# symek/facedeform

Hardware: AMD Instinct MI355X
Metric: deformed Mverts/sec at 256 ctrl pts, 1/2/4/8 MI355X vs host-CPU ref (higher is better)
Workload: dtype f32

## Files before the change

### facedeform_amd/csrc/fd_eval_shared.hip

```cpp
#include <cstdio>
#include <cstdlib>

#include <type_traits>

#include "fd_eval_common.h"
#include "fd_shared_common.h"

namespace fd {

namespace {


constexpr int kSharedThreads = 512;
constexpr int kWideWaves = 8;

constexpr bool shared_dense(int nF) { return nF > 12; }
constexpr int shared_tiles(int nF) { return shared_dense(nF) ? 3 * ((nF + 15) / 16) : (nF + 3) / 4; }
constexpr int shared_slots(int nT, bool dense) { return dense ? nT / 3 * 16 : nT * 4; }


struct SharedOut {
    float *P_out[kMaxBatch];
    float *falloff_out[kMaxBatch];
};

struct SharedParams {
    int64_t N;
    const float *P_in;
    const float *dist2;
    const float *tu, *tv, *nrm;
    float radius2, falloffrate;
    int ntiles;
    int nkb;
    int nF, nT;
    int kchunk;
    const MfmaTileH *ctiles;
    const float *norm;
    const uint4 *wtiles;
    const SharedFrame *frames;
    int fast;
    int delta;
    unsigned long long *stamps;
};

struct SharedSlots {
    const Rec32 *rec32[kMaxBatch];
    const DevModel *model[kMaxBatch];
    const double *centres[kMaxBatch];
    int M;
    int nreal;
    int *mismatch;
};

__device__ __forceinline__ bool rig_matches(const SharedSlots &slots, int f, int nF, int l, int per)
{
    bool same = true;
    if (f > 0 && f < nF && slots.centres[f] != slots.centres[0]) {
        const double *a = slots.centres[f], *b0 = slots.centres[0];
        const int n = 3 * slots.M;
        bool diff = false;
        int e = l;
        for (; e + 7 * per < n; e += 8 * per) {
            double va[8], vb[8];
#pragma unroll
            for (int u = 0; u < 8; ++u) { va[u] = a[e + u * per]; vb[u] = b0[e + u * per]; }
#pragma unroll
            for (int u = 0; u < 8; ++u) diff |= !(va[u] == vb[u]);
        }
        for (; e < n; e += per) diff |= !(a[e] == b0[e]);
        same = !diff;
    }
    for (int off = per / 2; off >= 1; off >>= 1) same = (__shfl_xor((int)same, off) != 0) && same;
    if (!same && l == 0 && slots.mismatch) *slots.mismatch = (f < slots.nreal ? f : slots.nreal - 1) + 1;
    return same;
}

__global__ __launch_bounds__(256) void k_pack_shared(const SharedSlots slots, const SharedOut out, int nF, int Mpad, int dense,
                                                      uint4 *wtiles, SharedFrame *frames, const MfmaTileH *ctiles, int gauss)
{
    const int kb = blockIdx.x, T = blockIdx.y, nT = gridDim.y, nkb = gridDim.x;
    if (T == 0 && gauss) {
        constexpr int per = (int)(sizeof(MfmaTileH) / 16);
        uint4 *dst = wtiles + (size_t)nkb * nT * 128 + (size_t)nT * 64;
        if (threadIdx.x < 32) {
            const int centre = 32 * kb + (int)threadIdx.x;
            dst[(size_t)2 * kb * per + threadIdx.x] =
                centre < Mpad ? *reinterpret_cast<const uint4 *>(&slots.rec32[0][centre]) : make_uint4(0u, 0u, 0u, 0u);
        }
        if (kb == 0 && threadIdx.x == 255) {
            const float *nn = slots.model[0]->norm32;
            dst[(size_t)2 * nkb * per] = make_uint4(__float_as_uint(nn[0]), __float_as_uint(nn[1]), __float_as_uint(nn[2]), __float_as_uint(nn[3]));
        }
    } else if (T == 0) {
        constexpr int per = (int)(sizeof(MfmaTileH) / 16);
        uint4 *dst = wtiles + (size_t)nkb * nT * 128 + (size_t)nT * 64;
        const int ntiles = Mpad / 16;
        if ((int)threadIdx.x < 2 * per) {
            const int tile = 2 * kb + (int)threadIdx.x / per;
            dst[(size_t)2 * kb * per + threadIdx.x] =
                tile < ntiles ? reinterpret_cast<const uint4 *>(ctiles + tile)[threadIdx.x % per] : make_uint4(0u, 0u, 0u, 0u);
        }
        if (kb == 0 && threadIdx.x == 255) {
            const float *nn = slots.model[0]->norm32;
            dst[(size_t)2 * nkb * per] = make_uint4(__float_as_uint(nn[0]), __float_as_uint(nn[1]), __float_as_uint(nn[2]), __float_as_uint(nn[3]));
        }
    }
    const int lane = threadIdx.x & 63, g = lane >> 4, rho = lane & 15;
    const int nfr = dense ? 16 : 4, f0 = dense ? 16 * (T / 3) : 4 * T;
    const int fi = dense ? rho : rho >> 2, c = dense ? T % 3 : rho & 3;
    __shared__ float s_scale[16];
    {
        const int per = 256 / nfr, q = threadIdx.x / per, l = threadIdx.x % per;
        const int f = f0 + q;
        float m = 0.f;
        if (f < nF) {
            m = slots.model[f]->wmax32;
        }
        for (int off = per / 2; off >= 1; off >>= 1) m = fmaxf(m, __shfl_xor(m, off));
        const bool same_rig = (kb == 0 && (!dense || T % 3 == 0)) ? rig_matches(slots, f, nF, l, per) : true;
        if (l == 0) {
            int k = 0;
            if (m > 0.f && m < INFINITY) k = 13 - (__builtin_amdgcn_frexp_expf(m) - 1);
            k = k < -100 ? -100 : (k > 100 ? 100 : k);
            s_scale[q] = ldexpf(1.f, k);
            if (kb == 0 && (!dense || T % 3 == 0)) {
                SharedFrame fr;
                fr.inv_scale = ldexpf(1.f, -k - (gauss ? kGaussShift : 0));
                fr.built = (f < nF && same_rig && slots.model[f]->terminationtype == 1) ? 1 : 0;
                fr.pad[0] = fr.pad[1] = 0;
                fr.P_out = f < nF ? out.P_out[f] : nullptr;
                fr.falloff_out = f < nF ? out.falloff_out[f] : nullptr;
                frames[f] = fr;
            }
        }
    }
    __syncthreads();
    if (threadIdx.x >= 64) return;
    const int f = f0 + fi;
    const float sc = s_scale[fi];
    f16x8 hi, lo;
#pragma unroll
    for (int sidx = 0; sidx < 8; ++sidx) {
        const int centre = 32 * kb + 16 * (sidx >> 2) + 4 * g + (sidx & 3);
        float w = 0.f;
        if (f < nF && c < 3 && centre < Mpad) {
            const Rec32 r = slots.rec32[f][centre];
            w = (c == 0 ? r.wx : (c == 1 ? r.wy : r.wz)) * sc;
        }
        const _Float16 h = (_Float16)w;
        hi[sidx] = h;
        lo[sidx] = (_Float16)(w - (float)h);
    }
    uint4 *dst = wtiles + ((size_t)kb * nT + T) * 128;
    dst[lane] = __builtin_bit_cast(uint4, hi);
    dst[64 + lane] = __builtin_bit_cast(uint4, lo);
// ... 764 lines not shown
                }
            }
            phi_half(nk - 1, 1, b1h, b1l);
            contract_half(nk - 1, 0, b0h, b0l);
            contract_half(nk - 1, 1, b1h, b1l);
        }

        FD_SSTAMP(1)
#pragma unroll
        for (int c = 0; c < NT; ++c) {
#pragma unroll
            for (int r = 0; r < 16; ++r) {
                const u32x2 sw = __builtin_amdgcn_permlane32_swap(__float_as_uint(acc[c][0][r]), __float_as_uint(acc[c][1][r]), false, false);
                acc[c][0][r] = __uint_as_float(sw[0]); acc[c][1][r] = __uint_as_float(sw[1]);
            }
        }
        const int64_t i = vbase + lane;
        const bool inb = i < p.N;
        const int64_t ic = inb ? i : p.N - 1;
        const bool gated = own_d2 > p.radius2;
        const unsigned off12 = 12u * (unsigned)lane, off4 = 4u * (unsigned)lane;
        if constexpr (!FAST) {
            nxt = load_raw(gu_next, fastTag);
        }
        auto row_of = [&](int fs, int c) -> float {
            const int row = 3 * fs + c, T = row / 32, rho = row % 32;
            return acc[T][(rho % 8) / 4][4 * (rho / 8) + rho % 4];
        };
        FD_SSTAMP(2)
        if constexpr (FAST) {
            const f32x4 ones = {1.f, 1.f, 1.f, 1.f};
            const unsigned voff = 12u * (unsigned)vbase + off12;
            const uint64_t fbase = 4ull * (uint64_t)vbase;
#pragma unroll
            for (int fs = 0; fs < NSLOT; ++fs) {
                const float inv = __uint_as_float((unsigned)__builtin_amdgcn_readlane((int)tab[(8 * fs) / 64], (8 * fs) % 64));
                const uint64_t pout = ((uint64_t)(unsigned)__builtin_amdgcn_readlane((int)tab[(8 * fs + 5) / 64], (8 * fs + 5) % 64) << 32) |
                                      (unsigned)__builtin_amdgcn_readlane((int)tab[(8 * fs + 4) / 64], (8 * fs + 4) % 64);
                const float d0 = row_of(fs, 0), d1 = row_of(fs, 1), d2c = row_of(fs, 2);
                if (fs % 4 == 0) __builtin_nontemporal_store(ones, (f32x4_a16 FD_GLOBAL *)(s_ftab[(fs / 4) * 64 + lane] + fbase));
                store_pos3_nt((Pos3 FD_GLOBAL *)((char FD_GLOBAL *)pout + voff), __builtin_fmaf(d0, inv, pos[0]), __builtin_fmaf(d1, inv, pos[1]),
                              __builtin_fmaf(d2c, inv, pos[2]));
            }
            settle(nxt);
            FD_SSTAMP(3)
            return;
        }
        if (inb && gated) {
            for (int f = 0; f < p.nF; ++f) {
                float *dstp = s_frames[f].P_out;
                if (p.delta) store_pos3((Pos3 FD_GLOBAL *)as_global(dstp) + i, 0.f, 0.f, 0.f);
                else if (dstp != p.P_in) store_pos3((Pos3 FD_GLOBAL *)as_global(dstp) + i, pos[0], pos[1], pos[2]);
            }
        }
        float fall = 1.f;
        float a1[3] = {0.f, 0.f, 0.f}, a2[3] = {0.f, 0.f, 0.f};
        const bool doit = inb && !gated;
        const float base[3] = {p.delta ? 0.f : pos[0], p.delta ? 0.f : pos[1], p.delta ? 0.f : pos[2]};
        if (doit) {
            if (p.dist2 != nullptr || !(p.radius2 != 0.f)) {
                const float q = fminf(own_d2 / p.radius2, 1.f);
                fall = powf(1.f - q, p.falloffrate);
            }
            if (p.tu) {
                float u[3] = {p.tu[3 * ic], p.tu[3 * ic + 1], p.tu[3 * ic + 2]};
                float v[3] = {p.tv[3 * ic], p.tv[3 * ic + 1], p.tv[3 * ic + 2]};
                float n[3] = {p.nrm[3 * ic], p.nrm[3 * ic + 1], p.nrm[3 * ic + 2]};
                normalize3(u[0], u[1], u[2]);
                normalize3(v[0], v[1], v[2]);
                normalize3(n[0], n[1], n[2]);
                float gm[3][3];
#pragma unroll
                for (int r = 0; r < 3; ++r)
#pragma unroll
                    for (int c = 0; c < 3; ++c) gm[r][c] = u[r] * u[c] + v[r] * v[c] + n[r] * n[c];
#pragma unroll
                for (int c = 0; c < 3; ++c) {
                    a1[c] = u[0] * gm[0][c] + u[1] * gm[1][c] + u[2] * gm[2][c];
                    a2[c] = v[0] * gm[0][c] + v[1] * gm[1][c] + v[2] * gm[2][c];
                }
                normalize3(a1[0], a1[1], a1[2]);
                normalize3(a2[0], a2[1], a2[2]);
            }
        }
#pragma unroll
        for (int fs = 0; fs < NSLOT; ++fs) {
            const int f = fs;
            if (f >= p.nF) continue;
            const float inv = __uint_as_float((unsigned)__builtin_amdgcn_readlane((int)tab[(8 * f) / 64], (8 * f) % 64));
            const bool built = __builtin_amdgcn_readlane((int)tab[(8 * f + 1) / 64], (8 * f + 1) % 64) != 0;
            const uint64_t pout = ((uint64_t)(unsigned)__builtin_amdgcn_readlane((int)tab[(8 * f + 5) / 64], (8 * f + 5) % 64) << 32) |
                                  (unsigned)__builtin_amdgcn_readlane((int)tab[(8 * f + 4) / 64], (8 * f + 4) % 64);
            const uint64_t fout = ((uint64_t)(unsigned)__builtin_amdgcn_readlane((int)tab[(8 * f + 7) / 64], (8 * f + 7) % 64) << 32) |
                                  (unsigned)__builtin_amdgcn_readlane((int)tab[(8 * f + 6) / 64], (8 * f + 6) % 64);
            if (!doit) continue;
            Pos3 FD_GLOBAL *dstP = (Pos3 FD_GLOBAL *)((char FD_GLOBAL *)(pout + 12ull * (uint64_t)vbase) + off12);
            if (!built) {
                if (p.delta) store_pos3(dstP, 0.f, 0.f, 0.f);
                else if (pout != (uint64_t)p.P_in) store_pos3(dstP, pos[0], pos[1], pos[2]);
                continue;
            }
            float disp[3] = {row_of(fs, 0) * inv, row_of(fs, 1) * inv, row_of(fs, 2) * inv};
            if (p.tu) {
                const float da1 = disp[0] * a1[0] + disp[1] * a1[1] + disp[2] * a1[2];
                const float da2 = disp[0] * a2[0] + disp[1] * a2[1] + disp[2] * a2[2];
#pragma unroll
                for (int c = 0; c < 3; ++c) disp[c] = a1[c] * da1 + a2[c] * da2;
            }
            if (fout) __builtin_nontemporal_store(fall, (float FD_GLOBAL *)((char FD_GLOBAL *)(fout + 4ull * (uint64_t)vbase) + off4));
            store_pos3_nt(dstP, base[0] + disp[0] * fall, base[1] + disp[1] * fall, base[2] + disp[2] * fall);
        }
        FD_SSTAMP(3)
    };
    bool built_here = true;
#pragma unroll
    for (int q = 0; q < kTabRegs; ++q) {
        const int idx = 64 * q + lane;
        if (idx < NSLOT * 8 && (idx & 7) == 1) built_here = built_here && tab[q] != 0u;
    }
    const bool fast_ok = p.fast && __all(built_here);
    const int nfull = (int)(p.N / THREADS);
    int u = dynamic ? next_unit(0) : wave;
    int ru = dynamic ? round_taken : 0;
    nxt = load_raw(unit_group(u) < ngroups ? unit_global(u) : 0, std::false_type{});
    settle(nxt);
    if (fast_ok) {
        while (unit_group(u) < nfull) {
            const int un = next_unit(u);
            const int run = dynamic ? round_taken : ru + 1;
            do_group(u, un, ru, std::true_type{});
            u = un; ru = run;
        }
    }
    while (unit_group(u) < ngroups) {
        const int un = next_unit(u);
        const int run = dynamic ? round_taken : ru + 1;
        do_group(u, un, ru, std::false_type{});
        u = un; ru = run;
    }
    if (stamp && lane == 0 && wave < 8) {
        for (int q = 0; q < 4; ++q) p.stamps[wave * 8 + q] = st_acc[q];
        p.stamps[wave * 8 + 4] = __builtin_amdgcn_s_memtime() - st_t0;
        p.stamps[wave * 8 + 5] = __builtin_amdgcn_s_memrealtime() - st_r0;
    }
    if (p.stamps != nullptr && lane == 0 && wave < 8 && blockIdx.x < kMaxCUs) {
        p.stamps[64 + ((size_t)blockIdx.x * 8 + wave) * 2] = st_r0;
        p.stamps[64 + ((size_t)blockIdx.x * 8 + wave) * 2 + 1] = __builtin_amdgcn_s_memrealtime();
    }
#undef FD_SSTAMP
}

constexpr int kW1Waves = 12;
constexpr int kW1Unit = 32;
constexpr size_t w1_fixed_lds(int nt) { return sizeof(SharedFrame) * (size_t)kWideSlots + 32 * 16 + (size_t)nt * 64 * 16 + 256 * sizeof(uint64_t) + 16; }

template <bool GAUSS, int NT, int NSLOT>
__global__ __launch_bounds__(64 * kW1Waves) __attribute__((amdgpu_waves_per_eu(kW1Waves / 4, kW1Waves / 4)))
void k_deform32_shared_w1(const SharedParams p, int ngroups)
{
    constexpr int WAVES = kW1Waves, THREADS = 64 * WAVES;
    constexpr int NLF = NSLOT / 2;
    constexpr int NFQ = (NSLOT + 7) / 8;
    static_assert(NSLOT % 4 == 0 && NSLOT <= kWideSlots && 3 * NLF <= 16 * NT, "frame slots in fours, three rows each, half of them per lane half");
    constexpr int kW16 = wide_w16(NT);
    extern __shared__ __attribute__((aligned(16))) char smem[];
    SharedFrame *s_frames = reinterpret_cast<SharedFrame *>(smem);
    uint4 *s_ptab = reinterpret_cast<uint4 *>(smem + sizeof(SharedFrame) * (size_t)kWideSlots);
    uint4 *s_poly = s_ptab + 32;
    uint64_t *s_ftab = reinterpret_cast<uint64_t *>(s_poly + NT * 64);
    unsigned *s_ticket = reinterpret_cast<unsigned *>(s_ftab + 256);
    uint4 *s_ct = reinterpret_cast<uint4 *>(s_ticket + 4);
    uint4 *s_w = s_ct + (size_t)64 * p.kchunk;
    const int tid = threadIdx.x;
    const int lane = tid & 63;
    const int wave = __builtin_amdgcn_readfirstlane(tid >> 6);
    const int h = lane >> 5, j = lane & 31;
    const float n0 = p.norm[0], n1 = p.norm[1], n2 = p.norm[2];
    const float inv_s = p.norm[3];
    f32x16 zero16;
#pragma unroll
    for (int r = 0; r < 16; ++r) zero16[r] = 0.f;

    auto stage_model = [&]() {
        const int nk = p.nkb;
        for (int q = tid; q < nk * 64; q += THREADS) s_ct[q] = reinterpret_cast<const uint4 *>(p.ctiles)[q];
        const u32x4 *src = reinterpret_cast<const u32x4 *>(p.wtiles);
        u32x4 *dst = reinterpret_cast<u32x4 *>(s_w);
        const int n16 = nk * kW16;
        int q = tid;
        for (; q + 7 * THREADS < n16; q += 8 * THREADS) {
            const u32x4 v0 = src[q], v1 = src[q + THREADS], v2 = src[q + 2 * THREADS], v3 = src[q + 3 * THREADS];
            const u32x4 v4 = src[q + 4 * THREADS], v5 = src[q + 5 * THREADS], v6 = src[q + 6 * THREADS], v7 = src[q + 7 * THREADS];
            dst[q] = v0; dst[q + THREADS] = v1; dst[q + 2 * THREADS] = v2; dst[q + 3 * THREADS] = v3;
            dst[q + 4 * THREADS] = v4; dst[q + 5 * THREADS] = v5; dst[q + 6 * THREADS] = v6; dst[q + 7 * THREADS] = v7;
        }
        for (; q < n16; q += THREADS) dst[q] = src[q];
        __syncthreads();
    };

    {
        const uint4 *src = reinterpret_cast<const uint4 *>(p.frames);
        uint4 *dst = reinterpret_cast<uint4 *>(s_frames);
        for (int q = tid; q < kWideSlots * (int)(sizeof(SharedFrame) / 16); q += THREADS) dst[q] = src[q];
        const uint4 *psrc = p.wtiles + (size_t)p.nkb * kW16;
        for (int q = tid; q < NT * 64; q += THREADS) s_poly[q] = psrc[q];
        if (tid == 0) *s_ticket = 0u;
        if (tid < 32) {
            const SharedFrame fr = p.frames[tid < NSLOT ? tid : NSLOT - 1];
            const uint64_t po = (uint64_t)fr.P_out;
            s_ptab[tid] = make_uint4((unsigned)po, (unsigned)(po >> 32), __float_as_uint(fr.inv_scale), (unsigned)fr.built);
        }
        if (p.fast && tid < NFQ * 64) {
            const int f = 8 * (tid >> 6) + ((tid & 63) >> 3);
            s_ftab[tid] = (uint64_t)p.frames[f < NSLOT ? f : NSLOT - 1].falloff_out + 16u * (unsigned)(tid & 7);
        }
    }
    stage_model();

    struct UnitRaw { float p[3]; float d2; };
    const int whole_rounds = ngroups / (int)gridDim.x;
    const int pool0 = whole_rounds * (int)gridDim.x * WAVES, total_units = ngroups * WAVES;
    auto unit_global = [&](int u) -> int {
        if (u < WAVES * whole_rounds) return ((int)blockIdx.x + (u / WAVES) * (int)gridDim.x) * WAVES + (u % WAVES);
        const int q = u - WAVES * whole_rounds;
        return q < 2 * WAVES ? pool0 + (int)blockIdx.x + q * (int)gridDim.x : total_units;
    };
    auto unit_group = [&](int u) -> int { const int g = unit_global(u); return g < total_units ? (g / WAVES) : ngroups; };
    auto next_unit = [&](int u) {
        (void)u;
        unsigned v = 0;
        if (lane == 0) v = __hip_atomic_fetch_add(s_ticket, 1u, __ATOMIC_RELAXED, __HIP_MEMORY_SCOPE_WORKGROUP);
        return (int)__builtin_amdgcn_readfirstlane(v);
    };
    auto load_raw = [&](int gu, auto fastTag) {
        constexpr bool FAST = decltype(fastTag)::value;
        UnitRaw r;
        const int64_t vi = (int64_t)gu * kW1Unit + j;
        const int64_t vc = vi < p.N ? vi : p.N - 1;
        if constexpr (FAST) {
            const char *pb = reinterpret_cast<const char *>(p.P_in) + (size_t)(12u * (unsigned)vc);
            r.p[0] = __builtin_nontemporal_load(reinterpret_cast<const float *>(pb)); r.p[1] = __builtin_nontemporal_load(reinterpret_cast<const float *>(pb + 4));
            r.p[2] = __builtin_nontemporal_load(reinterpret_cast<const float *>(pb + 8));
            r.d2 = 0.f;
        } else {
            r.p[0] = __builtin_nontemporal_load(&p.P_in[3 * vc]); r.p[1] = __builtin_nontemporal_load(&p.P_in[3 * vc + 1]);
            r.p[2] = __builtin_nontemporal_load(&p.P_in[3 * vc + 2]);
            r.d2 = p.dist2 ? p.dist2[vc] : 0.f;
        }
        return r;
    };
    auto settle = [&](const UnitRaw &r) { asm volatile("" :: "v"(r.p[0]), "v"(r.p[1]), "v"(r.p[2])); };
    UnitRaw nxt;
    int uc = 0;
#ifdef FD_TUNING
    const bool stamp = p.stamps != nullptr && blockIdx.x == 0;
    const unsigned long long st_t0 = p.stamps ? __builtin_amdgcn_s_memtime() : 0, st_r0 = p.stamps ? __builtin_amdgcn_s_memrealtime() : 0;
    unsigned long long st_prev = st_t0, st_acc[4] = {0, 0, 0, 0};
#define FD_W1STAMP(K) if (stamp) { __builtin_amdgcn_sched_barrier(0); const unsigned long long t_ = __builtin_amdgcn_s_memtime(); st_acc[K] += t_ - st_prev; st_prev = t_; __builtin_amdgcn_sched_barrier(0); }
#else
#define FD_W1STAMP(K)
#endif
    auto do_unit = [&](int u, int un, auto fastTag) {
        constexpr bool FAST = decltype(fastTag)::value;
        const int64_t vbase = (int64_t)unit_global(u) * kW1Unit;
        const int gu_next = unit_group(un) < ngroups ? unit_global(un) : unit_global(u);
        const UnitRaw cur = nxt;
        const float pos[3] = {cur.p[0], cur.p[1], cur.p[2]};
        const float own_d2 = cur.d2;
        f32x16 acc[NT];
        const float x = (cur.p[0] - n0) * inv_s, y = (cur.p[1] - n1) * inv_s, z = (cur.p[2] - n2) * inv_s;
        const bool lane_live = FAST ? true : ((vbase + j < p.N) && !(own_d2 > p.radius2));
        const float xx = __builtin_fmaf(z, z, __builtin_fmaf(y, y, x * x));
        f16x8 bop;
        {
            const float va = h == 0 ? -2.f * x : -2.f * z, vb2 = h == 0 ? -2.f * y : xx;
            const _Float16 ha = (_Float16)va, la = (_Float16)(va - (float)ha);
            const _Float16 hb = (_Float16)vb2, lb = (_Float16)(vb2 - (float)hb);
            const _Float16 one = (_Float16)1.0f;
            bop = h == 0 ? (f16x8){ha, la, ha, la, hb, lb, hb, lb} : (f16x8){ha, la, ha, la, one, one, hb, lb};
        }
        {
            constexpr float ps = GAUSS ? (float)(1 << kGaussShift) : 1.f;
            constexpr unsigned one16 = GAUSS ? 0x6400u : 0x3c00u;
            unsigned xyh, xyl, zxh, zxl;
            split_pair_f16(x * ps, y * ps, xyh, xyl);
            split_pair_f16(z * ps, xx * ps, zxh, zxl);
            u32x4 pb;
            if (h == 0) pb = (u32x4){one16 | (xyh << 16), (xyh >> 16) | (zxh << 16), (zxh >> 16) | (xyl << 16), (xyl >> 16) | (zxl << 16)};
            else pb = (u32x4){(zxl >> 16) | (one16 << 16), xyh, zxh, 0u};
            const f16x8 pbv = __builtin_bit_cast(f16x8, pb);
#pragma unroll
            for (int c = 0; c < NT; ++c)
                acc[c] = __builtin_amdgcn_mfma_f32_32x32x16_f16(__builtin_bit_cast(f16x8, s_poly[c * 64 + lane]), pbv, zero16, 0, 0, 0);
        }
        const bool wave_work = FAST ? true : __any(lane_live);
        if constexpr (FAST) nxt = load_raw(gu_next, fastTag);
        FD_W1STAMP(0)

        f32x16 dd;
        f16x8 w0h, w0l;
        auto d2_block = [&](int kb) {
            if constexpr (!GAUSS) dd = __builtin_amdgcn_mfma_f32_32x32x16_f16(__builtin_bit_cast(f16x8, s_ct[(size_t)kb * 64 + lane]), bop, zero16, 0, 0, 0);
        };
        auto phi_from = [&](int kb, u32x8 &xh, u32x8 &xl) {
            if constexpr (GAUSS) {
                const float4 *cr = reinterpret_cast<const float4 *>(s_ct + (size_t)kb * 64) + 4 * h;
#pragma unroll
                for (int q = 0; q < 8; ++q) {
                    float ph[2];
#pragma unroll
                    for (int e = 0; e < 2; ++e) {
                        const float4 c = cr[8 * (q >> 1) + 2 * (q & 1) + e];
                        const float dx = x - c.x, dy = y - c.y, dz = z - c.z;
                        float d2 = dx * dx;
                        d2 = __builtin_fmaf(dy, dy, d2);
                        d2 = __builtin_fmaf(dz, dz, d2);
                        ph[e] = __builtin_amdgcn_exp2f(__builtin_fmaf(d2, c.w, (float)kGaussShift));
                    }
                    unsigned hh, ll;
                    split_pair_f16<true>(ph[0], ph[1], hh, ll);
                    xh[q] = hh; xl[q] = ll;
                }
            } else {
#pragma unroll
                for (int q = 0; q < 8; ++q) {
                    unsigned hh, ll;
                    split_pair_f16<false, false>(d2_log_d2(dd[2 * q]), d2_log_d2(dd[2 * q + 1]), hh, ll);
                    xh[q] = hh; xl[q] = ll;
                }
                asm volatile("s_nop 1" : "+v"(xl[0]), "+v"(xl[1]), "+v"(xl[2]), "+v"(xl[3]), "+v"(xl[4]), "+v"(xl[5]), "+v"(xl[6]), "+v"(xl[7]));
            }
        };
        auto step = [&](int kb, int nk, const u32x8 &ch, const u32x8 &cl, u32x8 &nh, u32x8 &nl, auto lastTag) {
            constexpr bool LAST = decltype(lastTag)::value;
            constexpr int NP = 2 * NT;
            const uint4 *wk = s_w + (size_t)kb * kW16 + lane;
            const int kbn = kb + 1 < nk ? kb + 1 : kb, kbd = kb + 2 < nk ? kb + 2 : nk - 1;
            const uint4 *wkn = s_w + (size_t)kbn * kW16 + lane;
            if constexpr (!LAST) phi_from(kb + 1, nh, nl);
            f16x8 ph_ = w0h, pl_ = w0l;
#pragma unroll
            for (int pr = 0; pr < NP; ++pr) {
                const int s_ = pr / NT, c = pr % NT;
                f16x8 qh, ql;
                if (pr + 1 < NP) {
                    const int s2 = (pr + 1) / NT, c2 = (pr + 1) % NT;
                    qh = __builtin_bit_cast(f16x8, wk[((c2 * 2 + s2) * 2) * 64]); ql = __builtin_bit_cast(f16x8, wk[((c2 * 2 + s2) * 2 + 1) * 64]);
                } else {
                    qh = __builtin_bit_cast(f16x8, wkn[0]); ql = __builtin_bit_cast(f16x8, wkn[64]);
                }
                const f16x8 vh = __builtin_bit_cast(f16x8, (u32x4){ch[4 * s_], ch[4 * s_ + 1], ch[4 * s_ + 2], ch[4 * s_ + 3]});
                const f16x8 vl = __builtin_bit_cast(f16x8, (u32x4){cl[4 * s_], cl[4 * s_ + 1], cl[4 * s_ + 2], cl[4 * s_ + 3]});
                acc[c] = __builtin_amdgcn_mfma_f32_32x32x16_f16(ph_, vh, acc[c], 0, 0, 0);
                if constexpr (!LAST) if (pr == NP - 1) d2_block(kbd);
                acc[c] = __builtin_amdgcn_mfma_f32_32x32x16_f16(pl_, vh, acc[c], 0, 0, 0);
                acc[c] = __builtin_amdgcn_mfma_f32_32x32x16_f16(ph_, vl, acc[c], 0, 0, 0);
                ph_ = qh; pl_ = ql;
            }
            w0h = ph_; w0l = pl_;
            if constexpr (GAUSS || LAST) return;
            constexpr int NM = 6 * NT, TR2 = NT == 3 ? 0 : 8;
            constexpr int QD = 3 * (NP - 1);
#pragma unroll
            for (int q = 0; q < NM; ++q) {
                if (q < TR2) __builtin_amdgcn_sched_group_barrier(0x400, 2, 0);
                else if (q < TR2 + (16 - 2 * TR2)) __builtin_amdgcn_sched_group_barrier(0x400, 1, 0);
                __builtin_amdgcn_sched_group_barrier(0x008, 1, 0);
                if (q % 3 == 0) __builtin_amdgcn_sched_group_barrier(0x100, 2, 0);
                if (q == 1) __builtin_amdgcn_sched_group_barrier(0x100, 1, 0);
                if (q == QD) __builtin_amdgcn_sched_group_barrier(0x008, 1, 0);
                __builtin_amdgcn_sched_group_barrier(0x002, NT == 3 ? kW1Vpm : kW1Vpm + 1, 0);
            }
        };
        const bool k_loop = FAST || wave_work;
        if (k_loop) {
            const int nk = p.nkb;
            u32x8 ah_, al_, bh_, bl_;
            d2_block(0);
            phi_from(0, ah_, al_);
            d2_block(nk > 1 ? 1 : 0);
            w0h = __builtin_bit_cast(f16x8, s_w[lane]); w0l = __builtin_bit_cast(f16x8, s_w[64 + lane]);
            int kb = 0;
            while (kb + 2 < nk) {
                step(kb, nk, ah_, al_, bh_, bl_, std::false_type{});
                step(kb + 1, nk, bh_, bl_, ah_, al_, std::false_type{});
                kb += 2;
            }
            if (kb + 2 == nk) {
                step(kb, nk, ah_, al_, bh_, bl_, std::false_type{});
                step(kb + 1, nk, bh_, bl_, ah_, al_, std::true_type{});
            } else {
                step(kb, nk, ah_, al_, bh_, bl_, std::true_type{});
            }
        }

        auto accf = [&](int k) -> float { return acc[k / 16][k % 16]; };
        const int64_t i = vbase + j;
        FD_W1STAMP(1)
        if constexpr (!FAST) nxt = load_raw(gu_next, fastTag);
        if constexpr (FAST) {
            const f32x4 ones = {1.f, 1.f, 1.f, 1.f};
            uint64_t voff = 12ull * (uint64_t)i, fbase = 4ull * (uint64_t)vbase;
            asm volatile("" : "+v"(voff));
            uint4 ent[NLF];
            uint64_t fptr[NFQ];
#pragma unroll
            for (int lf = 0; lf < NLF; ++lf) ent[lf] = s_ptab[2 * lf + h];
#pragma unroll
            for (int q = 0; q < NFQ; ++q) fptr[q] = s_ftab[q * 64 + lane];
            __builtin_amdgcn_sched_group_barrier(0x100, NLF + NFQ, 0);
#pragma unroll
            for (int lf = 0; lf < NLF; ++lf) {
                const uint4 e = ent[lf];
                const uint64_t dst = (((uint64_t)e.y << 32) | (uint64_t)e.x) + voff;
                const float inv = __uint_as_float(e.z);
                if (lf % 4 == 0) __builtin_nontemporal_store(ones, (f32x4_a16 FD_GLOBAL *)(fptr[lf / 4] + fbase));
                store_pos3_nt((Pos3 FD_GLOBAL *)dst, __builtin_fmaf(accf(3 * lf), inv, pos[0]), __builtin_fmaf(accf(3 * lf + 1), inv, pos[1]),
                              __builtin_fmaf(accf(3 * lf + 2), inv, pos[2]));
            }
            settle(nxt);
            ++uc;
            FD_W1STAMP(2)
            return;
        }
        const bool inb = i < p.N;
        const int64_t ic = inb ? i : p.N - 1;
        const bool gated = own_d2 > p.radius2;
        if (inb && gated) {
            for (int f = h; f < p.nF; f += 2) {
                float *dstp = s_frames[f].P_out;
                if (p.delta) store_pos3((Pos3 FD_GLOBAL *)as_global(dstp) + i, 0.f, 0.f, 0.f);
                else if (dstp != p.P_in) store_pos3((Pos3 FD_GLOBAL *)as_global(dstp) + i, pos[0], pos[1], pos[2]);
            }
        }
        float fall = 1.f;
        float a1[3] = {0.f, 0.f, 0.f}, a2[3] = {0.f, 0.f, 0.f};
        const bool doit = inb && !gated;
        const float base[3] = {p.delta ? 0.f : pos[0], p.delta ? 0.f : pos[1], p.delta ? 0.f : pos[2]};
        if (doit) {
            if (p.dist2 != nullptr || !(p.radius2 != 0.f)) {
                const float q = fminf(own_d2 / p.radius2, 1.f);
                fall = powf(1.f - q, p.falloffrate);
            }
            if (p.tu) {
                float u3[3] = {p.tu[3 * ic], p.tu[3 * ic + 1], p.tu[3 * ic + 2]};
                float v3[3] = {p.tv[3 * ic], p.tv[3 * ic + 1], p.tv[3 * ic + 2]};
                float n3[3] = {p.nrm[3 * ic], p.nrm[3 * ic + 1], p.nrm[3 * ic + 2]};
                normalize3(u3[0], u3[1], u3[2]);
                normalize3(v3[0], v3[1], v3[2]);
                normalize3(n3[0], n3[1], n3[2]);
                float gm[3][3];
#pragma unroll
                for (int r = 0; r < 3; ++r)
#pragma unroll
                    for (int c = 0; c < 3; ++c) gm[r][c] = u3[r] * u3[c] + v3[r] * v3[c] + n3[r] * n3[c];
#pragma unroll
                for (int c = 0; c < 3; ++c) {
                    a1[c] = u3[0] * gm[0][c] + u3[1] * gm[1][c] + u3[2] * gm[2][c];
                    a2[c] = v3[0] * gm[0][c] + v3[1] * gm[1][c] + v3[2] * gm[2][c];
                }
                normalize3(a1[0], a1[1], a1[2]);
                normalize3(a2[0], a2[1], a2[2]);
            }
        }
#pragma unroll
        for (int lf = 0; lf < NLF; ++lf) {
            const int f = 2 * lf + h;
            if (f >= p.nF || !doit) continue;
            const SharedFrame fr = s_frames[f];
            Pos3 FD_GLOBAL *dstP = (Pos3 FD_GLOBAL *)as_global(fr.P_out) + i;
            if (!fr.built) {
                if (p.delta) store_pos3(dstP, 0.f, 0.f, 0.f);
                else if (fr.P_out != p.P_in) store_pos3(dstP, pos[0], pos[1], pos[2]);
                continue;
            }
            float disp[3] = {accf(3 * lf) * fr.inv_scale, accf(3 * lf + 1) * fr.inv_scale, accf(3 * lf + 2) * fr.inv_scale};
            if (p.tu) {
                const float da1 = disp[0] * a1[0] + disp[1] * a1[1] + disp[2] * a1[2];
                const float da2 = disp[0] * a2[0] + disp[1] * a2[1] + disp[2] * a2[2];
#pragma unroll
                for (int c = 0; c < 3; ++c) disp[c] = a1[c] * da1 + a2[c] * da2;
            }
            if (fr.falloff_out) __builtin_nontemporal_store(fall, (float FD_GLOBAL *)as_global(fr.falloff_out) + i);
            store_pos3_nt(dstP, base[0] + disp[0] * fall, base[1] + disp[1] * fall, base[2] + disp[2] * fall);
        }
    };
    bool built_here = true;
    if (lane < NSLOT) built_here = p.frames[lane].built != 0;
    const bool fast_ok = p.fast && __all(built_here);
    const int nfull = (int)(p.N / (kW1Unit * WAVES));
    int u = next_unit(0);
    nxt = load_raw(unit_group(u) < ngroups ? unit_global(u) : 0, std::false_type{});
    settle(nxt);
    if (fast_ok) {
        while (unit_group(u) < nfull) {
            const int un = next_unit(u);
            do_unit(u, un, std::true_type{});
            u = un;
        }
    }
    while (unit_group(u) < ngroups) {
        const int un = next_unit(u);
        do_unit(u, un, std::false_type{});
        u = un;
    }
#ifdef FD_TUNING
    if (stamp && lane == 0 && wave < 16) {
        for (int q = 0; q < 3; ++q) p.stamps[wave * 8 + q] = st_acc[q];
        p.stamps[wave * 8 + 3] = (unsigned long long)uc;
        p.stamps[wave * 8 + 4] = __builtin_amdgcn_s_memtime() - st_t0;
        p.stamps[wave * 8 + 5] = __builtin_amdgcn_s_memrealtime() - st_r0;
    }
#endif
#undef FD_W1STAMP
}
}

hipError_t launch_deform_shared(const SharedDeformArgs &a, hipStream_t stream)
{
    if (a.N <= 0 || a.nF <= 0) return hipSuccess;
    if (a.nF > kMaxBatch || a.Mpad % 16 != 0) return hipErrorInvalidValue;
    const int ntiles = a.Mpad / 16, nkb = (ntiles + 1) / 2;
    const bool gauss = a.kind != FD_KERNEL_THIN_PLATE;
    const bool wide = shared_wide(a.nF, a.kind);
    const bool dense = shared_dense(a.nF);
    const int nT = shared_tiles(a.nF);
    const int wslot = wide_slots(a.nF), wNT = wide_tiles(wslot);
    const int nslot = wide ? wslot : shared_slots(nT, dense);
    SharedSlots slots{};
    SharedOut out{};
    for (int f = 0; f < kMaxBatch; ++f) {
        const int q = f < a.nF ? f : a.nF - 1;
        slots.rec32[f] = a.rec32[q]; slots.model[f] = a.model[q]; slots.centres[f] = a.centres[q];
        out.P_out[f] = a.P_out[q]; out.falloff_out[f] = a.falloff_out ? a.falloff_out[q] : nullptr;
    }
    slots.M = a.M; slots.nreal = a.nF; slots.mismatch = a.mismatch;
    const bool w1 = wide && (kSharedLdsBudget - w1_fixed_lds(wNT)) / ((size_t)1024 + (size_t)wide_w16(wNT) * 16) >= (size_t)nkb;
    if (a.mode != 2) {
        if (wide)
            hipLaunchKernelGGL(k_pack_shared_wide, dim3(nkb, wNT), dim3(256), 0, stream, slots, out, a.nF, wslot, a.Mpad, (uint4 *)a.wtiles,
                               (SharedFrame *)a.frames, a.ctiles, gauss ? 1 : 0, w1 ? 1 : 0);
        else
            hipLaunchKernelGGL(k_pack_shared, dim3(nkb, nT), dim3(256), 0, stream, slots, out, nslot, a.Mpad, dense ? 1 : 0, (uint4 *)a.wtiles,
                               (SharedFrame *)a.frames, a.ctiles, gauss ? 1 : 0);
        if (a.packed_ev) {
            hipError_t e = hipEventRecord(a.packed_ev, stream);
            if (e != hipSuccess) return e;
        }
        if (a.mode == 1) return hipGetLastError();
    }
    SharedParams p{};
    p.N = a.N; p.P_in = a.P_in; p.dist2 = a.dist2; p.tu = a.tu; p.tv = a.tv; p.nrm = a.nrm;
    p.radius2 = a.radius2; p.falloffrate = a.falloffrate; p.delta = a.delta_out;
    p.ntiles = ntiles; p.nkb = nkb; p.nF = a.nF; p.nT = nT;
    if (wide) {
        const uint4 *copy = (const uint4 *)a.wtiles + (size_t)nkb * wide_w16(wNT) + (size_t)wNT * 64;
        p.ctiles = reinterpret_cast<const MfmaTileH *>(copy);
        p.norm = reinterpret_cast<const float *>(copy + (size_t)nkb * 64);
    } else {
        const uint4 *copy = (const uint4 *)a.wtiles + (size_t)nkb * nT * 128 + (size_t)nT * 64;
        p.ctiles = reinterpret_cast<const MfmaTileH *>(copy);
        p.norm = reinterpret_cast<const float *>(copy + (size_t)2 * nkb * (sizeof(MfmaTileH) / 16));
    }
    p.wtiles = (const uint4 *)a.wtiles; p.frames = (const SharedFrame *)a.frames;
    {
        bool fast = !a.delta_out && a.dist2 == nullptr && a.tu == nullptr && a.radius2 > 0.f && a.falloff_out != nullptr &&
                    a.N < ((int64_t)1 << 28) && 4 * (nslot - a.nF) <= a.nF;
        for (int f = 0; fast && f < a.nF; ++f) fast = a.falloff_out[f] != nullptr && a.P_out[f] != nullptr && ((uintptr_t)a.falloff_out[f] & 15) == 0;
        p.fast = fast ? 1 : 0;
    }
#ifdef FD_TUNING
    static unsigned long long *d_stamps = nullptr;
    static const bool want_stamps = tuning_env("FD_SHARED_STAMPS") != nullptr;
    constexpr size_t kStampWords = 64 + (size_t)kMaxCUs * 8 * 2;
    if (want_stamps && !d_stamps) (void)hipMalloc((void **)&d_stamps, kStampWords * sizeof(unsigned long long));
    if (want_stamps && d_stamps) (void)hipMemsetAsync(d_stamps, 0, kStampWords * sizeof(unsigned long long), stream);
    p.stamps = want_stamps ? d_stamps : nullptr;
#else
    p.stamps = nullptr;
#endif
    const size_t fixed = w1 ? w1_fixed_lds(wNT) :
                         wide ? sizeof(SharedFrame) * (size_t)kWideSlots + (size_t)wNT * 64 * 16 + 512 * sizeof(uint64_t) + 16
                              : sizeof(SharedFrame) * (size_t)shared_slots(nT, dense) + (size_t)nT * 64 * 16;
    const size_t per_kb = wide ? (size_t)1024 + (size_t)wide_w16(wNT) * 16 : 2 * sizeof(MfmaTileH) + (size_t)nT * 128 * 16;
    int kchunk = (int)((kSharedLdsBudget - fixed) / per_kb);
    if (kchunk < 1) return hipErrorInvalidValue;
    if (kchunk > nkb) kchunk = nkb;
    p.kchunk = kchunk;
    const size_t lds = fixed + per_kb * (size_t)kchunk;
    const int64_t per = w1 ? kW1Unit * kW1Waves : wide ? 64 * kWideWaves : kSharedThreads / 64 * 64;
    const int64_t ngroups = (a.N + per - 1) / per;
    const int64_t max_wgs = a.max_wgs > 0 ? (a.max_wgs < 4096 ? a.max_wgs : 4096) : (int64_t)device_cus();
    const unsigned grid = (unsigned)(ngroups < max_wgs ? ngroups : max_wgs);
#define FD_SHARED_CASE(NTV, DNS, GSS)                                                                                \
    {                                                                                                                \
        static LdsAttrOnce once;                                                                                     \
        hipError_t e = once.ensure((const void *)k_deform32_tps_shared<NTV, DNS, GSS>, 160 * 1024);                  \
        if (e != hipSuccess) return e;                                                                               \
        hipLaunchKernelGGL((k_deform32_tps_shared<NTV, DNS, GSS>), dim3(grid), dim3(kSharedThreads), lds, stream, p, (int)ngroups); \
    }
#define FD_SHARED_KIND(NTV, DNS) { if (gauss) FD_SHARED_CASE(NTV, DNS, true) else FD_SHARED_CASE(NTV, DNS, false) }
#define FD_WIDE_CASE(GSS, NTW, NSL)                                                                                  \
    {                                                                                                                \
        static LdsAttrOnce once;                                                                                     \
        hipError_t e = once.ensure((const void *)k_deform32_tps_shared_wide<GSS, NTW, NSL>, 160 * 1024); \
        if (e != hipSuccess) return e;                                                                               \
        hipLaunchKernelGGL((k_deform32_tps_shared_wide<GSS, NTW, NSL>), dim3(grid), dim3(64 * kWideWaves), lds, stream, p, (int)ngroups); \
    }
#define FD_WIDE_KIND(NTW, NSL) { if (gauss) FD_WIDE_CASE(true, NTW, NSL) else FD_WIDE_CASE(false, NTW, NSL) }
#define FD_W1_CASE(GSS, NTW, NSL)                                                                                    \
    {                                                                                                                \
        static LdsAttrOnce once;                                                                                     \
        hipError_t e = once.ensure((const void *)k_deform32_shared_w1<GSS, NTW, NSL>, 160 * 1024);                   \
        if (e != hipSuccess) return e;                                                                               \
        hipLaunchKernelGGL((k_deform32_shared_w1<GSS, NTW, NSL>), dim3(grid), dim3(64 * kW1Waves), lds, stream, p, (int)ngroups); \
    }
#define FD_W1_KIND(NTW, NSL) { if (gauss) FD_W1_CASE(true, NTW, NSL) else FD_W1_CASE(false, NTW, NSL) }
    if (w1) {
        if (wslot == 20) FD_W1_KIND(2, 20)
        else if (wslot == 24) FD_W1_KIND(3, 24)
        else if (wslot == 28) FD_W1_KIND(3, 28)
        else if (wslot == 32) FD_W1_KIND(3, 32)
        else return hipErrorInvalidValue;
    } else if (wide) {
        if (wslot == 20) FD_WIDE_KIND(2, 20)
        else if (wslot == 24) FD_WIDE_KIND(3, 24)
        else if (wslot == 28) FD_WIDE_KIND(3, 28)
        else if (wslot == 32) FD_WIDE_KIND(3, 32)
        else return hipErrorInvalidValue;
    } else if (dense) {
        if (nT == 3) FD_SHARED_KIND(3, true)
        else return hipErrorInvalidValue;
    } else {
        if (nT == 1) FD_SHARED_KIND(1, false)
        else if (nT == 2) FD_SHARED_KIND(2, false)
        else if (nT == 3) FD_SHARED_KIND(3, false)
        else return hipErrorInvalidValue;
    }
#undef FD_SHARED_KIND
#undef FD_SHARED_CASE
#undef FD_WIDE_CASE
#undef FD_WIDE_KIND
#undef FD_W1_CASE
#undef FD_W1_KIND
#ifdef FD_TUNING
    if (want_stamps && d_stamps) {
        static unsigned long long h[kStampWords];
        (void)hipStreamSynchronize(stream);
        if (hipMemcpy(h, d_stamps, sizeof(h), hipMemcpyDeviceToHost) == hipSuccess) {
            if (w1) {
                fprintf(stderr, "[w1 stamps, shader cycles per wave of workgroup 0: load+poly | K loop | epilogue | units | whole (counts, 100 MHz ticks)]\n");
                for (int w = 0; w < kW1Waves; ++w)
                    fprintf(stderr, "   wave %2d: %8llu %8llu %8llu  units %llu  whole %llu counts in %llu ticks = %.3f GHz\n", w, h[w * 8], h[w * 8 + 1], h[w * 8 + 2], h[w * 8 + 3],
                            h[w * 8 + 4], h[w * 8 + 5], h[w * 8 + 5] ? (double)h[w * 8 + 4] / (double)h[w * 8 + 5] * 0.1 : 0.0);
            } else if (wide) {
                unsigned long long t0 = ~0ull, t1 = 0;
                const unsigned sgrid = grid < kMaxCUs ? grid : kMaxCUs;
                for (unsigned b = 0; b < sgrid * 8; ++b) if (h[64 + 2 * b]) { t0 = h[64 + 2 * b] < t0 ? h[64 + 2 * b] : t0; t1 = h[65 + 2 * b] > t1 ? h[65 + 2 * b] : t1; }
                fprintf(stderr, "[shared stamps: %u workgroups, first entry to last exit %.1f us; per workgroup (entry, exit) in us after the first entry:]\n", grid, (t1 - t0) * 0.01);
                for (unsigned b = 0; b < sgrid; ++b) {
                    unsigned long long a = ~0ull, z = 0;
                    for (int w = 0; w < 8; ++w) if (h[64 + 2 * (b * 8 + w)]) { a = h[64 + 2 * (b * 8 + w)] < a ? h[64 + 2 * (b * 8 + w)] : a; z = h[65 + 2 * (b * 8 + w)] > z ? h[65 + 2 * (b * 8 + w)] : z; }
                    fprintf(stderr, "%s%5.1f-%5.1f", b % 8 ? "  " : "\n   ", (a - t0) * 0.01, (z - t0) * 0.01);
                }
                fprintf(stderr, "\n");
            }
            if (!w1) fprintf(stderr, "[shared stamps, shader cycles per wave of workgroup 0: load+poly | K loop | transposes | per-vertex + frames]\n");
            for (int w = 0; w < 8 && !w1; ++w)
                fprintf(stderr, "   wave %d: %8llu %8llu %8llu %8llu   (whole: %llu counts in %llu reference ticks)\n", w, h[w * 8], h[w * 8 + 1], h[w * 8 + 2], h[w * 8 + 3],
                        h[w * 8 + 4], h[w * 8 + 5]);
        }
    }
#endif
    return hipGetLastError();
}

size_t shared_wtile_bytes(int Mpad, int nF)
{
    const int nkb = (Mpad / 16 + 1) / 2, nT = shared_tiles(nF);
    return (size_t)nkb * nT * 128 * 16 + (size_t)nT * 64 * 16 + (size_t)2 * nkb * sizeof(MfmaTileH) + 16;
}
const char *shared_kernel_name(int Mpad, int nF, int kind)
{
    if (!shared_wide(nF, kind)) return "k_deform32_tps_shared";
    const int nkb = (Mpad / 16 + 1) / 2, wNT = wide_tiles(wide_slots(nF));
    const bool w1 = (kSharedLdsBudget - w1_fixed_lds(wNT)) / ((size_t)1024 + (size_t)wide_w16(wNT) * 16) >= (size_t)nkb;
    return w1 ? "k_deform32_shared_w1" : "k_deform32_tps_shared_wide";
}
SharedPacking shared_packing(int Mpad, int nF)
{
    SharedPacking q{};
    const int nkb = (Mpad / 16 + 1) / 2;
    if (!shared_wide(nF, 0)) {
        const int nT = shared_tiles(nF);
        q.layout = shared_dense(nF) ? 1 : 0;
        q.ntiles = nT;
        q.poly_at = (size_t)nkb * nT * 128;
        q.copy_at = q.poly_at + (size_t)nT * 64;
        q.norm_at = q.copy_at + (size_t)2 * nkb * (sizeof(MfmaTileH) / 16);
    } else {
        const int wNT = wide_tiles(wide_slots(nF));
        const bool w1 = (kSharedLdsBudget - w1_fixed_lds(wNT)) / ((size_t)1024 + (size_t)wide_w16(wNT) * 16) >= (size_t)nkb;
        q.layout = w1 ? 3 : 2;
        q.ntiles = wNT;
        q.poly_at = (size_t)nkb * wide_w16(wNT);
        q.copy_at = q.poly_at + (size_t)wNT * 64;
        q.norm_at = q.copy_at + (size_t)nkb * 64;
    }
    return q;
}
size_t shared_frame_bytes(int nF)
{
    return sizeof(SharedFrame) * (size_t)shared_slots(shared_tiles(nF), shared_dense(nF));
}

}
```

Before: 63760.

## Overlap first vertex load with single-pass batched staging of w1 tables

Restructures the w1 kernel prologue: each wave now statically takes its first unit (ticket starts at WAVES) and issues its vertex load before staging, and all table loads (frames, pointer/falloff tables, poly, ctiles, first 8 weight chunks) are issued into registers before any LDS store, with a single barrier. The built flag is read from LDS instead of global memory. This aims to shorten the per-workgroup prologue latency by overlapping global loads. Also adds tuning-only per-wave timing stamps and a summary printout.

```diff
diff --git a/facedeform_amd/csrc/fd_eval_shared.hip b/facedeform_amd/csrc/fd_eval_shared.hip
--- a/facedeform_amd/csrc/fd_eval_shared.hip
+++ b/facedeform_amd/csrc/fd_eval_shared.hip
@@ -1,6 +1,9 @@
 #include <cstdio>
 #include <cstdlib>
 
+#ifdef FD_TUNING
+#include <algorithm>
+#endif
 #include <type_traits>
 
 #include "fd_eval_common.h"
@@ -1071,6 +1074,7 @@
 
 constexpr int kW1Waves = 12;
 constexpr int kW1Unit = 32;
+constexpr size_t kW1StampBase = 128;
 constexpr size_t w1_fixed_lds(int nt) { return sizeof(SharedFrame) * (size_t)kWideSlots + 32 * 16 + (size_t)nt * 64 * 16 + 256 * sizeof(uint64_t) + 16; }
 
 template <bool GAUSS, int NT, int NSLOT>
@@ -1094,47 +1098,15 @@
     const int lane = tid & 63;
     const int wave = __builtin_amdgcn_readfirstlane(tid >> 6);
     const int h = lane >> 5, j = lane & 31;
+#ifdef FD_TUNING
+    const unsigned long long st_in = p.stamps ? __builtin_amdgcn_s_memrealtime() : 0;
+#endif
     const float n0 = p.norm[0], n1 = p.norm[1], n2 = p.norm[2];
     const float inv_s = p.norm[3];
     f32x16 zero16;
 #pragma unroll
     for (int r = 0; r < 16; ++r) zero16[r] = 0.f;
 
-    auto stage_model = [&]() {
-        const int nk = p.nkb;
-        for (int q = tid; q < nk * 64; q += THREADS) s_ct[q] = reinterpret_cast<const uint4 *>(p.ctiles)[q];
-        const u32x4 *src = reinterpret_cast<const u32x4 *>(p.wtiles);
-        u32x4 *dst = reinterpret_cast<u32x4 *>(s_w);
-        const int n16 = nk * kW16;
-        int q = tid;
-        for (; q + 7 * THREADS < n16; q += 8 * THREADS) {
-            const u32x4 v0 = src[q], v1 = src[q + THREADS], v2 = src[q + 2 * THREADS], v3 = src[q + 3 * THREADS];
-            const u32x4 v4 = src[q + 4 * THREADS], v5 = src[q + 5 * THREADS], v6 = src[q + 6 * THREADS], v7 = src[q + 7 * THREADS];
-            dst[q] = v0; dst[q + THREADS] = v1; dst[q + 2 * THREADS] = v2; dst[q + 3 * THREADS] = v3;
-            dst[q + 4 * THREADS] = v4; dst[q + 5 * THREADS] = v5; dst[q + 6 * THREADS] = v6; dst[q + 7 * THREADS] = v7;
-        }
-        for (; q < n16; q += THREADS) dst[q] = src[q];
-        __syncthreads();
-    };
-
-    {
-        const uint4 *src = reinterpret_cast<const uint4 *>(p.frames);
-        uint4 *dst = reinterpret_cast<uint4 *>(s_frames);
-        for (int q = tid; q < kWideSlots * (int)(sizeof(SharedFrame) / 16); q += THREADS) dst[q] = src[q];
-        const uint4 *psrc = p.wtiles + (size_t)p.nkb * kW16;
-        for (int q = tid; q < NT * 64; q += THREADS) s_poly[q] = psrc[q];
-        if (tid == 0) *s_ticket = 0u;
-        if (tid < 32) {
-            const SharedFrame fr = p.frames[tid < NSLOT ? tid : NSLOT - 1];
-            const uint64_t po = (uint64_t)fr.P_out;
-            s_ptab[tid] = make_uint4((unsigned)po, (unsigned)(po >> 32), __float_as_uint(fr.inv_scale), (unsigned)fr.built);
-        }
-        if (p.fast && tid < NFQ * 64) {
-            const int f = 8 * (tid >> 6) + ((tid & 63) >> 3);
-            s_ftab[tid] = (uint64_t)p.frames[f < NSLOT ? f : NSLOT - 1].falloff_out + 16u * (unsigned)(tid & 7);
-        }
-    }
-    stage_model();
 
     struct UnitRaw { float p[3]; float d2; };
     const int whole_rounds = ngroups / (int)gridDim.x;
@@ -1171,7 +1143,52 @@
     auto settle = [&](const UnitRaw &r) { asm volatile("" :: "v"(r.p[0]), "v"(r.p[1]), "v"(r.p[2])); };
     UnitRaw nxt;
     int uc = 0;
+
+    int u = wave;
+    nxt = load_raw(unit_group(u) < ngroups ? unit_global(u) : 0, std::false_type{});
+    {
+        static_assert(NT * 64 <= THREADS && kWideSlots * (int)(sizeof(SharedFrame) / 16) <= THREADS && NFQ * 64 <= THREADS, "one table entry per thread");
+        constexpr int NREC = kWideSlots * (int)(sizeof(SharedFrame) / 16);
+        const int nk = p.nkb, nct = nk * 64, n16 = nk * kW16;
+        const uint4 *fsrc = reinterpret_cast<const uint4 *>(p.frames);
+        const uint4 *psrc = p.wtiles + (size_t)nk * kW16;
+        const uint4 *csrc = reinterpret_cast<const uint4 *>(p.ctiles);
+        const u32x4 *wsrc = reinterpret_cast<const u32x4 *>(p.wtiles);
+        u32x4 *wdst = reinterpret_cast<u32x4 *>(s_w);
+        const int ff = 8 * (tid >> 6) + ((tid & 63) >> 3);
+        const uint4 r_rec = fsrc[tid < NREC ? tid : 0];
+        const SharedFrame r_fr = p.frames[(tid & 31) < NSLOT ? (tid & 31) : NSLOT - 1];
+        const uint64_t r_fall = (uint64_t)p.frames[(tid < NFQ * 64 && ff < NSLOT) ? ff : NSLOT - 1].falloff_out;
+        const uint4 r_poly = psrc[tid < NT * 64 ? tid : 0];
+        const uint4 r_ct = csrc[tid < nct ? tid : 0];
+        u32x4 w[8];
+#pragma unroll
+        for (int k = 0; k < 8; ++k) { const int q = tid + k * THREADS; w[k] = wsrc[q < n16 ? q : n16 - 1]; }
+        if (tid == 0) *s_ticket = (unsigned)WAVES;
+        if (tid < NREC) reinterpret_cast<uint4 *>(s_frames)[tid] = r_rec;
+        if (tid < 32) {
+            const uint64_t po = (uint64_t)r_fr.P_out;
+            s_ptab[tid] = make_uint4((unsigned)po, (unsigned)(po >> 32), __float_as_uint(r_fr.inv_scale), (unsigned)r_fr.built);
+        }
+        if (p.fast && tid < NFQ * 64) s_ftab[tid] = r_fall + 16u * (unsigned)(tid & 7);
+        if (tid < NT * 64) s_poly[tid] = r_poly;
+        if (tid < nct) s_ct[tid] = r_ct;
+#pragma unroll
+        for (int k = 0; k < 8; ++k) { const int q = tid + k * THREADS; if (q < n16) wdst[q] = w[k]; }
+        for (int q = tid + THREADS; q < nct; q += THREADS) s_ct[q] = csrc[q];
+        for (int q0 = tid + 8 * THREADS; q0 < n16; q0 += 8 * THREADS) {
+#pragma unroll
+            for (int k = 0; k < 8; ++k) { const int q = q0 + k * THREADS; w[k] = wsrc[q < n16 ? q : n16 - 1]; }
+#pragma unroll
+            for (int k = 0; k < 8; ++k) { const int q = q0 + k * THREADS; if (q < n16) wdst[q] = w[k]; }
+        }
+        __syncthreads();
+    }
+    bool built_here = true;
+    if (lane < NSLOT) built_here = s_frames[lane].built != 0;
+    settle(nxt);
 #ifdef FD_TUNING
+    const unsigned long long st_first = p.stamps ? __builtin_amdgcn_s_memrealtime() : 0;
     const bool stamp = p.stamps != nullptr && blockIdx.x == 0;
     const unsigned long long st_t0 = p.stamps ? __builtin_amdgcn_s_memtime() : 0, st_r0 = p.stamps ? __builtin_amdgcn_s_memrealtime() : 0;
     unsigned long long st_prev = st_t0, st_acc[4] = {0, 0, 0, 0};
@@ -1404,13 +1421,8 @@
             store_pos3_nt(dstP, base[0] + disp[0] * fall, base[1] + disp[1] * fall, base[2] + disp[2] * fall);
         }
     };
-    bool built_here = true;
-    if (lane < NSLOT) built_here = p.frames[lane].built != 0;
     const bool fast_ok = p.fast && __all(built_here);
     const int nfull = (int)(p.N / (kW1Unit * WAVES));
-    int u = next_unit(0);
-    nxt = load_raw(unit_group(u) < ngroups ? unit_global(u) : 0, std::false_type{});
-    settle(nxt);
     if (fast_ok) {
         while (unit_group(u) < nfull) {
             const int un = next_unit(u);
@@ -1429,6 +1441,10 @@
         p.stamps[wave * 8 + 3] = (unsigned long long)uc;
         p.stamps[wave * 8 + 4] = __builtin_amdgcn_s_memtime() - st_t0;
         p.stamps[wave * 8 + 5] = __builtin_amdgcn_s_memrealtime() - st_r0;
+    }
+    if (p.stamps != nullptr && lane == 0 && blockIdx.x < kMaxCUs) {
+        unsigned long long *s = p.stamps + kW1StampBase + ((size_t)blockIdx.x * WAVES + wave) * 3;
+        s[0] = st_in; s[1] = st_first; s[2] = __builtin_amdgcn_s_memrealtime();
     }
 #endif
 #undef FD_W1STAMP
@@ -1491,7 +1507,7 @@
 #ifdef FD_TUNING
     static unsigned long long *d_stamps = nullptr;
     static const bool want_stamps = tuning_env("FD_SHARED_STAMPS") != nullptr;
-    constexpr size_t kStampWords = 64 + (size_t)kMaxCUs * 8 * 2;
+    constexpr size_t kStampWords = kW1StampBase + (size_t)kMaxCUs * kW1Waves * 3;
     if (want_stamps && !d_stamps) (void)hipMalloc((void **)&d_stamps, kStampWords * sizeof(unsigned long long));
     if (want_stamps && d_stamps) (void)hipMemsetAsync(d_stamps, 0, kStampWords * sizeof(unsigned long long), stream);
     p.stamps = want_stamps ? d_stamps : nullptr;
@@ -1572,6 +1588,34 @@
                 for (int w = 0; w < kW1Waves; ++w)
                     fprintf(stderr, "   wave %2d: %8llu %8llu %8llu  units %llu  whole %llu counts in %llu ticks = %.3f GHz\n", w, h[w * 8], h[w * 8 + 1], h[w * 8 + 2], h[w * 8 + 3],
                             h[w * 8 + 4], h[w * 8 + 5], h[w * 8 + 5] ? (double)h[w * 8 + 4] / (double)h[w * 8 + 5] * 0.1 : 0.0);
+                const unsigned sgrid = grid < kMaxCUs ? grid : kMaxCUs;
+                static double ramp[kMaxCUs], skew[kMaxCUs], pro[kMaxCUs * kW1Waves], steady[kMaxCUs * kW1Waves];
+                unsigned long long t0 = ~0ull, t1 = 0;
+                for (unsigned b = 0; b < sgrid * kW1Waves; ++b) {
+                    const unsigned long long *s = h + kW1StampBase + 3 * (size_t)b;
+                    if (s[0]) { t0 = s[0] < t0 ? s[0] : t0; t1 = s[2] > t1 ? s[2] : t1; }
+                }
+                size_t nw = 0, nb = 0;
+                for (unsigned b = 0; b < sgrid; ++b) {
+                    unsigned long long a = ~0ull, z = 0;
+                    for (int w = 0; w < kW1Waves; ++w) {
+                        const unsigned long long *s = h + kW1StampBase + 3 * ((size_t)b * kW1Waves + w);
+                        if (!s[0]) continue;
+                        a = s[0] < a ? s[0] : a; z = s[2] > z ? s[2] : z;
+                        pro[nw] = (s[1] - s[0]) * 0.01; steady[nw] = (s[2] - s[1]) * 0.01; ++nw;
+                    }
+                    if (z) { ramp[nb] = (a - t0) * 0.01; skew[nb] = (t1 - z) * 0.01; ++nb; }
+                }
+                auto stat = [](double *v, size_t n, double &med, double &mx) {
+                    med = mx = 0.0;
+                    if (!n) return;
+                    std::sort(v, v + n);
+                    med = v[n / 2]; mx = v[n - 1];
+                };
+                double m[4], x[4];
+                stat(ramp, nb, m[0], x[0]); stat(pro, nw, m[1], x[1]); stat(steady, nw, m[2], x[2]); stat(skew, nb, m[3], x[3]);
+                fprintf(stderr, "[w1 split, us, %u workgroups, %d frames: first entry to last exit %.2f | ramp median %.2f max %.2f | prologue median %.2f max %.2f | "
+                                "steady median %.2f max %.2f | skew median %.2f max %.2f]\n", grid, a.nF, (t1 - t0) * 0.01, m[0], x[0], m[1], x[1], m[2], x[2], m[3], x[3]);
             } else if (wide) {
                 unsigned long long t0 = ~0ull, t1 = 0;
                 const unsigned sgrid = grid < kMaxCUs ? grid : kMaxCUs;
```

After: 64040, median of 6. About the same (+0.4%).
